# DaehwanKimLab/centrifuge

Hardware: NVIDIA H100
Metric: reads/sec (100 bp SE classification) (higher is better)
Workload: dtype u64

## Files before the change

### centrifuge_b200/capi.py

```python
import ctypes as C
import os

import numpy as np

HERE = os.path.dirname(os.path.abspath(__file__))
LIB_PATH = os.path.join(HERE, "libcfb200.so")

CFB_UID_NONE = 0xFFFFFFFF
REC_DTYPE = np.dtype([("taxid", "<u8"), ("score", "<u4"), ("hitlen", "<u4"), ("uid", "<u4"), ("pad", "<u4")])

_lib = None


class CfbError(RuntimeError):
    pass


class IndexInfo(C.Structure):
    _fields_ = [("len", C.c_uint64), ("num_sides", C.c_uint64), ("n_seqs", C.c_uint64), ("n_tax_nodes", C.c_uint64),
                ("n_boundaries", C.c_uint64), ("line_rate", C.c_int32), ("off_rate", C.c_int32), ("ftab_chars", C.c_int32),
                ("sample_bytes", C.c_int32), ("compressed", C.c_int32), ("device", C.c_int32), ("device_bytes", C.c_uint64)]


class IndexTables(C.Structure):
# ... 280 lines not shown
        out = (C.c_uint64 * 5)()
        _ck(lib().cfb_ctx_requests(self.h, out))
        return dict(zip(["rank16", "ftab2", "ftabk", "walk8", "ftabd"], [int(x) for x in out]))

    def request_breakdown(self):
        out = (C.c_uint64 * 8)()
        _ck(lib().cfb_ctx_request_breakdown(self.h, out))
        names = ["rank16_w1", "rank16_w2_4", "rank16_w5", "walk8_try_row", "walk8_ok_row", "walk8_try_range", "walk8_ok_range", "walk8_ok_w5"]
        return dict(zip(names, [int(x) for x in out]))

    def search_iter_stats(self):
        out = (C.c_uint64 * 8)()
        _ck(lib().cfb_ctx_search_iter_stats(self.h, out))
        names = ["warp_iters", "lane_requests", "consumer_paths", "restart_paths", "task_iters", "clk_head", "clk_wait", "clk_tail"]
        return dict(zip(names, [int(x) for x in out]))

    def counters(self):
        out = (C.c_uint64 * 8)()
        _ck(lib().cfb_ctx_counters(self.h, out))
        names = ["units", "partial_searches", "ftab_probes", "sides_search", "walk_steps", "rows_resolved", "lf_steps", "ext_searches"]
        return dict(zip(names, [int(x) for x in out]))

    def launches(self):
        n = C.c_uint64()
        _ck(lib().cfb_ctx_kernel_launches(self.h, C.byref(n)))
        return int(n.value)

    def close(self):
        if self.h:
            lib().cfb_ctx_destroy(self.h)
# ... 133 lines not shown
```

### centrifuge_b200/csrc/cf_logic.h

```cpp
#ifndef CF_LOGIC_H_
#define CF_LOGIC_H_

#include <stdint.h>

#ifdef __CUDACC__
#define CFB_HD __host__ __device__ __forceinline__
#define CFB_HDN __host__ __device__
#else
#define CFB_HD inline
#define CFB_HDN inline
#endif

namespace cfb {

static const uint64_t kOff = 0xffffffffffffffffull;
static const uint64_t kUnk = 0xfffffffffffffffeull;
static const uint32_t kBwNone = 0xffffffffu;

struct IndexView {
	const uint64_t* sides;
	const uint64_t* ftab;
	const uint64_t* eftab;
	const uint16_t* sample16;
	const uint32_t* sample32;
	const uint64_t* brow;
	const uint32_t* bseq;
	const uint32_t* bbits;
	const uint64_t* seq_taxid;
	const int32_t*  seq_path;
	const uint64_t* paths;
	const uint8_t*  seq_excluded;
	const uint64_t* host_taxids;
	const uint64_t* rank16;
	const uint64_t* ftab2;
	const uint16_t* rtab16;
	const uint32_t* rtab32;
	const uint64_t* ftabk;
	const uint64_t* walk8;
	uint64_t walk8_rows;
	int32_t  ftabd_chars;
	uint64_t len, zoff, zside, fchr[4], last_boundary, num_sides;
	uint32_t zoffc, n_boundaries, n_seqs, n_host;
	int32_t  off_rate, ftab_chars, bshift, ftabk_chars;
};

struct Params {
	uint32_t khits, min_hitlen, ihits, increment;
	uint32_t tree_traverse, class_rank_slot;
};

struct HitRec { uint64_t top, bot; uint32_t bwoff, len; };

static const uint64_t kRowMask = (1ull << 40) - 1ull, kRowStart = 1ull << 63, kRowSameTs = 1ull << 58;

struct Counters {
	unsigned long long units, partial_searches, ftab_probes, sides_search, walk_steps, rows_resolved, lf_steps, ext_searches;
	unsigned long long req_rank16, req_ftab2, req_ftabk, req_walk8, req_ftabd;
	unsigned long long r16_w1, r16_w2_4, r16_w5, w8_try_row, w8_ok_row, w8_try_range, w8_ok_range, w8_ok_w5;
	unsigned long long it_warp, it_lane_req, it_consumers, it_restarts, it_task, clk_head, clk_wait, clk_tail;
};

CFB_HD int popc64(uint64_t x) {
#ifdef __CUDA_ARCH__
	return __popcll(x);
#else
	return __builtin_popcountll(x);
#endif
}
CFB_HD uint32_t ctz32(uint32_t x) {
#ifdef __CUDA_ARCH__
	return (uint32_t)(__ffs(x) - 1);
#else
	return (uint32_t)__builtin_ctz(x);
#endif
// ... 361 lines not shown
			const uint64_t nelt = hsize(L[hi]) < maxG ? hsize(L[hi]) : maxG;
			if(nelt > p.ihits) continue;
			const uint64_t head = kRowStart | ((uint64_t)(L[hi].len & 0xffffu) << 40) | ((uint64_t)(rdi & 1) << 56) | ((uint64_t)(fwi & 1) << 57)
			                    | (ts == last_ts ? kRowSameTs : 0ull);
			last_ts = ts;
			for(uint64_t e = 0; e < nelt; e++) out[k++] = ((L[hi].top + e) & kRowMask) | (e == 0 ? head : 0ull);
			cnt += nelt;
			if(cnt >= maxG) break;
		}
	}
};

static const uint32_t kUidOff = 0xffffffffu;
struct Entry {
	uint64_t taxID;
	uint32_t uniqueID;
	uint32_t scores[2][2], lens[2][2];
	uint32_t score, hitlen, ts;
	int32_t  pid;
	uint8_t  rank;
	uint8_t  pad[3];
};
struct TaxCnt { uint32_t count; uint32_t pad; uint64_t parent; };
struct TaxCntLess { CFB_HD bool operator()(const TaxCnt& a, const TaxCnt& b) const { return a.count < b.count || (a.count == b.count && a.parent < b.parent); } };

struct OutRec { uint64_t taxid; uint32_t score, hitlen, uid, pad; };

CFB_HD bool is_host(const IndexView& v, uint64_t taxid) {
	uint32_t lo = 0, hi = v.n_host;
	while(lo < hi) { uint32_t mid = (lo + hi) >> 1; if(v.host_taxids[mid] < taxid) lo = mid + 1; else hi = mid; }
	return lo < v.n_host && v.host_taxids[lo] == taxid;
}
CFB_HD uint32_t path_size(const Entry& e) { return e.pid < 0 ? 0u : 10u; }
CFB_HD uint64_t path_at(const IndexView& v, const Entry& e, uint32_t i) { return v.paths[(uint64_t)e.pid * 10 + i]; }

CFB_HDN uint32_t score_plan(const IndexView& v, const Params& p, const uint64_t* rows, const uint32_t* ids, uint64_t n, Entry* map) {
	uint32_t nmap = 0, ts = 0;
	for(uint64_t k = 0; k < n;) {
		const uint64_t head = rows[k];
		if(!(head & kRowSameTs)) ts++;
		const uint64_t hl = (head >> 40) & 0xffffu; const int rdi = (int)((head >> 56) & 1), fwi = (int)((head >> 57) & 1);
		uint64_t nelt = 1;
		while(k + nelt < n && !(rows[k + nelt] & kRowStart)) nelt++;
		const uint32_t* my = ids + k; k += nelt;
		const uint32_t sc = (uint32_t)((hl - 15) * (hl - 15));
		for(uint64_t e = 0; e < nelt; e++) {
			const uint32_t ref = my[e];
			bool dup = false;
			for(uint64_t q = 0; q < e; q++) if(my[q] == ref) { dup = true; break; }
			if(dup) continue;
			uint64_t taxID = ref < v.n_seqs ? v.seq_taxid[ref] : 0;
			if(v.seq_excluded && ref < v.n_seqs && v.seq_excluded[ref]) continue;
			const int32_t pid = ref < v.n_seqs ? v.seq_path[ref] : -1;
			uint8_t rank = (uint8_t)p.class_rank_slot;
			if(rank > 0 && pid >= 0) {
				for(; rank < 10; rank++) { const uint64_t t = v.paths[(uint64_t)pid * 10 + rank]; if(t != 0) { taxID = t; break; } }
			}
			uint32_t idx = 0;
			for(; idx < nmap; ++idx) {
				const bool same = rank == 0 ? (ref == map[idx].uniqueID) : (taxID == map[idx].taxID);
				if(same) {
					if(map[idx].ts != ts) { map[idx].scores[rdi][fwi] += sc; map[idx].lens[rdi][fwi] += (uint32_t)hl; map[idx].ts = ts; }
					break;
				}
			}
			if(idx >= nmap) {
				Entry& n2 = map[nmap++];
				n2.uniqueID = ref; n2.taxID = taxID;
				n2.scores[0][0] = n2.scores[0][1] = n2.scores[1][0] = n2.scores[1][1] = 0;
				n2.lens[0][0] = n2.lens[0][1] = n2.lens[1][0] = n2.lens[1][1] = 0;
				n2.scores[rdi][fwi] = sc; n2.lens[rdi][fwi] = (uint32_t)hl;
				n2.score = 0; n2.hitlen = 0; n2.ts = ts; n2.pid = pid; n2.rank = rank;
			}
		}
	}
	return nmap;
}


CFB_HDN uint32_t reduce_and_emit(const IndexView& v, const Params& p, bool paired, Entry* map, uint32_t nmap,
                                 TaxCnt* tc, OutRec* out) {
	const uint32_t k = p.khits;
	for(uint32_t i = 0; i < nmap; i++) {
		Entry& h = map[i];
		const uint32_t s0 = h.scores[0][0] > h.scores[0][1] ? h.scores[0][0] : h.scores[0][1];
		const uint32_t l0 = h.lens[0][0] > h.lens[0][1] ? h.lens[0][0] : h.lens[0][1];
		if(paired) {
			const uint32_t s1 = h.scores[1][0] > h.scores[1][1] ? h.scores[1][0] : h.scores[1][1];
			const uint32_t l1 = h.lens[1][0] > h.lens[1][1] ? h.lens[1][0] : h.lens[1][1];
			h.score = s0 + s1; h.hitlen = l0 + l1;
		} else { h.score = s0; h.hitlen = l0; }
	}
	int64_t best = 0; bool only_host = false;
	for(uint32_t i = 0; i < nmap; i++) {
		if((int64_t)map[i].score > best) { best = map[i].score; only_host = is_host(v, map[i].taxID); }
		else if((int64_t)map[i].score == best) only_host |= is_host(v, map[i].taxID);
	}
	if(!only_host && nmap > k) {
		uint32_t bs = map[0].score;
		for(uint32_t i = 1; i < nmap; i++) if(bs < map[i].score) bs = map[i].score;
		for(int i = 0; i < (int)nmap; i++) {
			if(map[i].score < bs) { if(i + 1 < (int)nmap) map[i] = map[nmap - 1]; nmap--; i--; }
		}
		if(!p.tree_traverse && nmap > k) return 0;
		uint8_t rank = 0;
		while(nmap > k) {
			uint32_t ntc = 0;
			for(uint32_t i = 0; i < nmap; i++) {
				Entry& h = map[i];
				while(h.rank < rank) {
					if((uint32_t)h.rank + 1 >= path_size(h)) { h.rank = 255; break; }
					h.rank += 1; h.taxID = path_at(v, h, h.rank);
				}
				if(h.rank > rank) continue;
				const uint64_t parent = ((uint32_t)rank + 1 >= path_size(h)) ? 1 : path_at(v, h, rank + 1);
				if(parent == 0) continue;
				uint32_t j = 0;
				for(; j < ntc; j++) if(tc[j].parent == parent) { tc[j].count += 1; break; }
				if(j == ntc) { tc[ntc].count = 1; tc[ntc].pad = 0; tc[ntc].parent = parent; ntc++; }
			}
			if(ntc == 0) {
				if(rank < path_size(map[0])) { rank++; continue; } else break;
			}
			ss_heapsort(tc, tc + ntc, TaxCntLess());
			uint32_t j = ntc;
			while(j-- > 0) {
				const uint64_t parent = tc[j].parent;
				for(uint32_t i = 0; i < nmap; i++) {
					Entry& h = map[i];
					if(h.rank != rank) continue;
					const uint64_t cur_parent = ((uint32_t)rank + 1 >= path_size(h)) ? 1 : path_at(v, h, rank + 1);
					if(parent == cur_parent) { h.uniqueID = kUidOff; h.rank = rank + 1; h.taxID = parent; }
				}
				bool first = true;
				for(uint32_t i = 0; i < nmap; i++) {
					if(parent == map[i].taxID) {
						if(!first) { if(i + 1 < nmap) map[i] = map[nmap - 1]; nmap--; i--; }
						else first = false;
					}
				}
				if(nmap <= k) break;
			}
			++rank;
			if(rank > path_size(map[0])) break;
		}
	}
	if(!only_host && nmap > k) return 0;
// ... 34 lines not shown
```

### centrifuge_b200/csrc/cf_multi.cuh

```cuda
#include <dlfcn.h>
#include <nccl.h>

extern "C" int cfb_ctx_count_records(cfb_ctx* c, int on) {
	if(!c) return fail(CFB_EINVAL, "null ctx");
	CK(cudaSetDevice(c->ix->device));
	if(on) { int rc = counts_init(c); if(rc) return rc; }
	c->fold_records = on != 0;
	return CFB_OK;
}
extern "C" int cfb_counts_taxids(cfb_ctx* c, uint64_t* taxid, uint64_t cap, uint64_t* n) {
	if(!c || !n) return fail(CFB_EINVAL, "null argument");
	CK(cudaSetDevice(c->ix->device));
	int rc = counts_init(c); if(rc) return rc;
	*n = c->cnt.n;
	if(taxid) { if(cap < c->cnt.n) return fail(CFB_EINVAL, "cfb_counts_taxids: buffer too small"); memcpy(taxid, c->cnt.h_taxid.data(), (size_t)c->cnt.n * 8); }
	return CFB_OK;
}
extern "C" int cfb_counts_reset(cfb_ctx* c) {
	if(!c) return fail(CFB_EINVAL, "null ctx");
	CK(cudaSetDevice(c->ix->device));
	if(!c->cnt.ready) return CFB_OK;
	CK(cudaDeviceSynchronize());
	CK(cudaMemset(c->cnt.total.p, 0, 3ull * c->cnt.n * 8)); CK(cudaMemset(c->cnt.global.p, 0, 3ull * c->cnt.n * 8));
	c->cnt.reduced = false;
// ... 145 lines not shown
	if(!c || !out) return fail(CFB_EINVAL, "null argument");
	CK(cudaSetDevice(c->ix->device));
	Counters h; CK(cudaMemcpy(&h, c->d_ctr, sizeof h, cudaMemcpyDeviceToHost));
	out[0] = h.r16_w1; out[1] = h.r16_w2_4; out[2] = h.r16_w5;
	out[3] = h.w8_try_row; out[4] = h.w8_ok_row; out[5] = h.w8_try_range; out[6] = h.w8_ok_range; out[7] = h.w8_ok_w5;
	return CFB_OK;
}
extern "C" int cfb_ctx_search_iter_stats(cfb_ctx* c, uint64_t out[8]) {
	if(!c || !out) return fail(CFB_EINVAL, "null argument");
	CK(cudaSetDevice(c->ix->device));
	Counters h; CK(cudaMemcpy(&h, c->d_ctr, sizeof h, cudaMemcpyDeviceToHost));
	out[0] = h.it_warp; out[1] = h.it_lane_req; out[2] = h.it_consumers; out[3] = h.it_restarts; out[4] = h.it_task;
	out[5] = h.clk_head; out[6] = h.clk_wait; out[7] = h.clk_tail;
	return CFB_OK;
}

__device__ __forceinline__ uint64_t gmix(uint64_t x) { x += 0x9E3779B97F4A7C15ull; x = (x ^ (x >> 30)) * 0xBF58476D1CE4E5B9ull; x = (x ^ (x >> 27)) * 0x94D049BB133111EBull; return x ^ (x >> 31); }
template <int W, int ILP>
__global__ void __launch_bounds__(128) k_gather_probe(const unsigned long long* __restrict__ a, uint64_t n, uint32_t iters, unsigned long long* sink) {
	const uint64_t tid = (uint64_t)blockIdx.x * blockDim.x + threadIdx.x;
	uint64_t h = gmix(tid * 0x2545F4914F6CDD1Dull + 1), acc = 0;
	for(uint32_t it = 0; it < iters; it++) {
		unsigned long long v[ILP][W];
		#pragma unroll
		for(int k = 0; k < ILP; k++) {
			h = gmix(h + k);
			const uint64_t u = h % n;
			if(W == 2) { const ulonglong2 q = __ldg(reinterpret_cast<const ulonglong2*>(a) + u); v[k][0] = q.x; v[k][W - 1] = q.y; }
			else v[k][0] = __ldg(a + u);
		}
// ... 42 lines not shown
```

### centrifuge_b200/csrc/cfb200.cu

```cuda
#include "../../include/cfb200.h"
#include "cf_index.h"
#include "cf_kernels.cuh"

#include <algorithm>
#include <atomic>
#include <mutex>
#include <thread>
#include <fcntl.h>
#include <unistd.h>
#include <cstdarg>
#include <cstdio>
#include <cstring>
#include <set>
#include <string>
#include <vector>

using namespace cfb;

enum { M_DONE = 0, M_FTAB = 1, M_LF = 2, M_NEED = 3, M_FTABK = 4, M_TASK = 5 };

struct SearchArgs {
	IndexView v; Params p; BatchView b;
	HitRec* hits; uint32_t* nhits; uint32_t cap;
	unsigned long long* task_ctr64; uint32_t ntasks, chunk;
// ... 594 lines not shown
	}
	const unsigned lane = threadIdx.x & 31;
	uint64_t incl = rows;
	for(int d = 1; d < 32; d <<= 1) { const uint64_t t = __shfl_up_sync(0xffffffffu, incl, d); if((int)lane >= d) incl += t; }
	const uint64_t warp_total = __shfl_sync(0xffffffffu, incl, 31);
	unsigned long long base = 0;
	if(lane == 31 && warp_total) base = atomicAdd(a.row_total, (unsigned long long)warp_total);
	base = __shfl_sync(0xffffffffu, base, 31);
	if(!live) return;
	const uint64_t off = base + incl - rows;
	a.nrows[unit] = (uint32_t)rows; a.row_off[unit] = off;
	if(rows && off + rows <= a.rows_cap) { EmitRows er(a.p, u, a.rows + off); for_each_visit(a.p, u, er); }
}

static const int kScoreThreads = 128;
static const uint32_t kScorePool = 128;
static const uint32_t kNoSlot = 0xffffffffu;
template <int MINB>
__global__ void __launch_bounds__(kScoreThreads, MINB) k_score(const UnitArgs a) {
	__shared__ uint64_t s_rows[kScorePool]; __shared__ uint32_t s_ids[kScorePool];
	__shared__ Entry s_map[kScorePool]; __shared__ TaxCnt s_tc[kScorePool]; __shared__ OutRec s_recs[kScorePool];
	__shared__ uint32_t s_used;
	if(threadIdx.x == 0) s_used = 0;
	__syncthreads();
	const uint32_t unit = blockIdx.x * blockDim.x + threadIdx.x;
	const unsigned lane = threadIdx.x & 31;
	const bool valid = unit < a.b.n_units;
	const bool fits = *a.row_total <= a.rows_cap;
	const uint64_t n = valid && fits ? a.nrows[unit] : 0, off = valid && fits ? a.row_off[unit] : 0;
	const uint64_t base = __shfl_sync(0xffffffffu, off, 0);
	uint64_t span = n ? off + n - base : 0;
	for(int d = 16; d > 0; d >>= 1) span = max(span, __shfl_xor_sync(0xffffffffu, span, d));
	uint32_t slot = kNoSlot;
	if(lane == 0 && span) {
		uint32_t cur = *(volatile uint32_t*)&s_used;
		while(span <= kScorePool - cur) {
			const uint32_t old = atomicCAS(&s_used, cur, cur + (uint32_t)span);
			if(old == cur) { slot = cur; break; }
			cur = old;
		}
	}
	slot = __shfl_sync(0xffffffffu, slot, 0);
	const bool sh = slot != kNoSlot;
	if(sh) {
		for(uint32_t j = lane; j < (uint32_t)span; j += 32) { s_rows[slot + j] = a.rows[base + j]; s_ids[slot + j] = a.ids[base + j]; }
		__syncwarp();
	}
	const uint32_t loc = sh ? slot + (uint32_t)(off - base) : 0u;
	uint32_t no = 0;
	if(n > 0) {
		const uint8_t fl = a.b.flags ? a.b.flags[unit] : 3;
		int mates = 0;
		for(int m = 0; m < a.b.n_mates; m++) if(((fl >> m) & 1) && (m ? a.b.len[1][unit] : a.b.len[0][unit]) != 0) mates++;
		const uint64_t* rows = sh ? s_rows + loc : a.rows + off;
		const uint32_t* ids = sh ? s_ids + loc : a.ids + off;
		Entry* map = sh ? s_map + loc : a.entries + off;
		TaxCnt* tc = sh ? s_tc + loc : a.tcs + off;
		OutRec* out = sh ? s_recs + loc : a.recs_sparse + off;
		const uint32_t nmap = score_plan(a.v, a.p, rows, ids, n, map);
		no = reduce_and_emit(a.v, a.p, mates == 2, map, nmap, tc, out);
	}
	if(valid) a.nout[unit] = no;
	if(sh) {
		__syncwarp();
		for(int u = 0; u < 32; u++) {
			const uint32_t cnt = __shfl_sync(0xffffffffu, no, u) * 3u, l = __shfl_sync(0xffffffffu, loc, u);
			const uint64_t o = __shfl_sync(0xffffffffu, off, u);
			const uint64_t* src = reinterpret_cast<const uint64_t*>(s_recs + l);
			uint64_t* dst = reinterpret_cast<uint64_t*>(a.recs_sparse + o);
			for(uint32_t w = lane; w < cnt; w += 32) dst[w] = src[w];
		}
	}
}

static const int kScanBlock = 256, kScanPer = 4;

__global__ void __launch_bounds__(kScanBlock) k_scan_sums(const uint32_t* in, uint64_t n, uint64_t* bsum) {
	__shared__ uint64_t sh[kScanBlock];
	const uint64_t base = (uint64_t)blockIdx.x * kScanBlock * kScanPer + (uint64_t)threadIdx.x * kScanPer;
	uint64_t s = 0;
	for(int i = 0; i < kScanPer; i++) if(base + i < n) s += in[base + i];
	sh[threadIdx.x] = s; __syncthreads();
	for(int d = kScanBlock / 2; d > 0; d >>= 1) { if((int)threadIdx.x < d) sh[threadIdx.x] += sh[threadIdx.x + d]; __syncthreads(); }
	if(threadIdx.x == 0) bsum[blockIdx.x] = sh[0];
}
__global__ void k_scan_top(uint64_t* bsum, uint64_t nb, uint64_t* total) {
	__shared__ uint64_t carry;
// ... 380 lines not shown
	if(!p) return;
	memset(p, 0, sizeof *p); p->khits = 5; p->min_hitlen = 22; p->tree_traverse = 1; p->class_rank_slot = 0;
}

static const int kSlots = 17;

struct Slot {
	cudaStream_t st = nullptr;
	cudaEvent_t ev[6] = {nullptr, nullptr, nullptr, nullptr, nullptr, nullptr};
	HBuf<uint8_t> h_bases; HBuf<uint64_t> h_off; HBuf<uint32_t> h_len; HBuf<uint8_t> h_flags;
	DBuf<uint8_t> d_bases; DBuf<uint64_t> d_off; DBuf<uint32_t> d_len; DBuf<uint8_t> d_flags;
	HBuf<uint64_t> h_words; DBuf<uint64_t> d_words, d_npos, d_woff; DBuf<uint32_t> d_wlen;
	DBuf<uint64_t> pk; DBuf<uint32_t> nm;
	DBuf<HitRec> hits; DBuf<uint32_t> nhits; DBuf<HitRec> regen; DBuf<uint32_t> regen_n; uint64_t regen_slots = 0; uint32_t full_cap = 0; DBuf<uint32_t> nrows; DBuf<uint64_t> row_off; DBuf<uint64_t> bsum;
	DBuf<uint64_t> rows; DBuf<uint32_t> ids; DBuf<Entry> entries; DBuf<TaxCnt> tcs; DBuf<OutRec> sparse;
	DBuf<uint32_t> nout; DBuf<uint64_t> out_off; DBuf<OutRec> dense; DBuf<uint32_t> rec_off32;
	DBuf<unsigned long long> scal;
	HBuf<unsigned long long> h_scal;
	HBuf<OutRec> h_recs; HBuf<uint32_t> h_rec_off;
	DBuf<unsigned long long> cnt;
	bool folded = false, is_text = false, commit_pending = false;
	BatchView bv; uint64_t n_units = 0, n_bases = 0; uint32_t maxlen = 0, cap = 0; uint64_t rows_cap = 0, dense_cap = 0;
	bool pending = false, reran = false;
	bool want_host = false; uint64_t d2h_recs = 0;
	void release() {
		h_bases.release(); h_off.release(); h_len.release(); h_flags.release(); d_bases.release(); d_off.release(); d_len.release(); d_flags.release();
		h_words.release(); d_words.release(); d_npos.release(); d_woff.release(); d_wlen.release();
		pk.release(); nm.release(); hits.release(); nhits.release(); regen.release(); regen_n.release(); nrows.release(); row_off.release(); bsum.release(); rows.release(); ids.release(); entries.release(); tcs.release();
		sparse.release(); nout.release(); out_off.release(); dense.release(); rec_off32.release(); scal.release(); h_scal.release(); h_recs.release(); h_rec_off.release(); cnt.release();
		for(int i = 0; i < 6; i++) if(ev[i]) cudaEventDestroy(ev[i]);
		if(st) cudaStreamDestroy(st);
	}
};

struct cfb_dbatch { int slot; uint64_t n_units; };
struct TextCtx;
static void text_release(cfb_ctx*);
static void comm_release(cfb_ctx*);

struct CountsCtx {
	bool ready = false;
	std::vector<uint64_t> h_taxid; DBuf<uint64_t> d_taxid; uint32_t n = 0;
	DBuf<unsigned long long> total, global; bool reduced = false;
	void release() { d_taxid.release(); total.release(); global.release(); }
};

struct cfb_ctx {
	const cfb_index* ix = nullptr;
	IndexView view; Params prm;
	DBuf<uint8_t> d_excl; DBuf<uint64_t> d_host;
	Slot slots[kSlots];
	Counters* d_ctr = nullptr; int count = 0;
	uint64_t launches = 0;
	int resolve_blocks = 0;
	cfb_dbatch resident; bool resident_used = false;
	double rec_ratio = 2.0;
	uint64_t rows_cap0 = 0;
	TextCtx* text = nullptr;
	CountsCtx cnt; bool fold_records = false;
	bool keep_short = false;
	uint64_t regen_lists = 0, regen_tasks = 0;
	uint64_t regen_slots0 = 0;
	void* comm = nullptr; int comm_rank = 0, comm_size = 1; cudaStream_t comm_st = nullptr;
};

// ... 10 lines not shown
			t = nd->parent;
		}
	}
}

extern "C" void cfb_ctx_destroy(cfb_ctx* c) {
	if(!c) return;
	if(c->ix && c->ix->device >= 0) cudaSetDevice(c->ix->device);
	if(getenv("CFB_REGEN_STATS") && c->regen_tasks)
		fprintf(stderr, "[cfb] strand lists regenerated by k_prep: %llu of %llu (%.3f %%)\n", (unsigned long long)c->regen_lists,
		        (unsigned long long)c->regen_tasks, 100.0 * (double)c->regen_lists / (double)c->regen_tasks);
	text_release(c);
	comm_release(c);
	c->cnt.release();
	for(int i = 0; i < kSlots; i++) c->slots[i].release();
	c->d_excl.release(); c->d_host.release();
	if(c->d_ctr) cudaFree(c->d_ctr);
	delete c;
}

extern "C" int cfb_ctx_create(const cfb_index* ix, const cfb_params* p, cfb_ctx** out) {
	if(!ix || !p || !out) return fail(CFB_EINVAL, "cfb_ctx_create: null argument");
	if(ix->device < 0) return fail(CFB_ENODEV, "index was loaded host-only; classification needs a CUDA device (no CPU fallback)");
	if(p->khits < 1) return fail(CFB_EINVAL, "khits must be >= 1");
	CK(cudaSetDevice(ix->device));
	cfb_ctx* c = new cfb_ctx();
	c->ix = ix; c->view = ix->view;
	const HostIndex& h = ix->h;
	Params& q = c->prm;
	q.khits = (uint32_t)p->khits;
	q.min_hitlen = (uint32_t)(p->min_hitlen < 15 ? 15 : p->min_hitlen);
	q.ihits = (uint32_t)std::max(p->khits, 5) * (h.compressed ? 4u : 40u);
	q.increment = (2 * q.min_hitlen <= 33) ? 10 : (2 * q.min_hitlen - 33);
	q.tree_traverse = p->tree_traverse ? 1 : 0;
	q.class_rank_slot = (uint32_t)(p->class_rank_slot & 0xff);
	std::set<uint64_t> host, excl;
	expand_taxids(h, p->host_taxids, p->n_host_taxids, host);
	expand_taxids(h, p->excluded_taxids, p->n_excluded_taxids, excl);
	#define CKC(call) do { cudaError_t e_ = (call); if(e_ != cudaSuccess) { cfb_ctx_destroy(c); return fail(CFB_ECUDA, "%s failed: %s", #call, cudaGetErrorString(e_)); } } while(0)
	if(!excl.empty()) {
		std::vector<uint8_t> fl(h.seq_taxid.size(), 0);
		for(size_t i = 0; i < fl.size(); i++) fl[i] = excl.count(h.seq_taxid[i]) ? 1 : 0;
		CKC(c->d_excl.ensure(fl.size())); CKC(cudaMemcpy(c->d_excl.p, fl.data(), fl.size(), cudaMemcpyHostToDevice));
		c->view.seq_excluded = c->d_excl.p;
	}
	if(!host.empty()) {
		std::vector<uint64_t> hv(host.begin(), host.end());
		CKC(c->d_host.ensure(hv.size())); CKC(cudaMemcpy(c->d_host.p, hv.data(), hv.size() * 8, cudaMemcpyHostToDevice));
		c->view.host_taxids = c->d_host.p; c->view.n_host = (uint32_t)hv.size();
	}
	for(int i = 0; i < kSlots; i++) {
		CKC(cudaStreamCreateWithFlags(&c->slots[i].st, cudaStreamNonBlocking));
		for(int e = 0; e < 6; e++) CKC(cudaEventCreate(&c->slots[i].ev[e]));
		CKC(c->slots[i].scal.ensure(8)); CKC(c->slots[i].h_scal.ensure(8));
	}
	CKC(cudaMalloc((void**)&c->d_ctr, sizeof(Counters))); CKC(cudaMemset(c->d_ctr, 0, sizeof(Counters)));
	cudaDeviceSetLimit(cudaLimitMaxL2FetchGranularity, 32);
	cudaGetLastError();
	int occ = 0;
// ... 212 lines not shown
	const SearchKernel search = search_kernel(s.maxlen, c->count);
	const bool keep_short = search == k_search_long<true> || search == k_search_long<false> || c->prm.min_hitlen < kLongLen || c->keep_short;
	if(stage == 0) {
		if(s.cap == 0) {
			s.full_cap = s.maxlen / 4 + 8;
			s.cap = keep_short ? s.full_cap : s.maxlen / kLongLen + 2;
		}
		CK(s.hits.ensure(ntasks * s.cap)); CK(s.nhits.ensure(ntasks));
		if(!keep_short) {
			s.regen_slots = std::max<uint64_t>(s.regen_slots, c->regen_slots0 ? c->regen_slots0 : std::max<uint64_t>(ntasks / 32, 1024));
			CK(s.regen.ensure(s.regen_slots * s.full_cap)); CK(s.regen_n.ensure(s.regen_slots));
			CK(cudaMemsetAsync(s.scal.p + 6, 0, sizeof(unsigned long long), s.st));
		}
		const uint32_t W = (s.maxlen + 31) / 32 + 1;
		CK(s.pk.ensure(ntasks * W + 2)); CK(s.nm.ensure(ntasks * W + 2)); CK(s.nrows.ensure(n)); CK(s.row_off.ensure(n + 1));
		CK(s.bsum.ensure(scan_blocks + 1)); CK(s.nout.ensure(n)); CK(s.out_off.ensure(n + 1)); CK(s.rec_off32.ensure(n + 1));
		s.rows_cap = std::max<uint64_t>(s.rows_cap, c->rows_cap0 ? c->rows_cap0 : std::max<uint64_t>(n * 12, 4096));
	}
	CK(s.rows.ensure(s.rows_cap)); CK(s.ids.ensure(s.rows_cap)); CK(s.entries.ensure(s.rows_cap)); CK(s.tcs.ensure(s.rows_cap)); CK(s.sparse.ensure(s.rows_cap));
	s.dense_cap = s.rows_cap; CK(s.dense.ensure(s.dense_cap));
	CK(cudaMemsetAsync(s.scal.p, 0, 4 * sizeof(unsigned long long), s.st));
	if(time_it) CK(cudaEventRecord(s.ev[0], s.st));
	Counters* ctr = c->count ? c->d_ctr : nullptr;
	if(c->count && stage == 0) CK(cudaMemsetAsync(c->d_ctr, 0, sizeof(Counters), s.st));
	UnitArgs ua; ua.v = c->view; ua.p = c->prm; ua.b = s.bv; ua.hits = s.hits.p; ua.nhits = s.nhits.p; ua.cap = s.cap;
	ua.nrows = s.nrows.p; ua.row_off = s.row_off.p; ua.row_total = s.scal.p + 3; ua.rows = s.rows.p; ua.ids = s.ids.p; ua.rows_cap = s.rows_cap;
	ua.entries = s.entries.p; ua.tcs = s.tcs.p; ua.recs_sparse = s.sparse.p; ua.nout = s.nout.p;
	ua.overflow = (unsigned int*)(s.scal.p + 2); ua.ctr = ctr;
	ua.regen = s.regen.p; ua.regen_n = s.regen_n.p; ua.regen_ctr = s.scal.p + 6; ua.regen_slots = s.regen_slots; ua.full_cap = s.full_cap; ua.keep_short = keep_short ? 1u : 0u;
	if(stage == 0) {
		SearchArgs sa; sa.v = c->view; sa.p = c->prm; sa.b = s.bv; sa.hits = s.hits.p; sa.nhits = s.nhits.p; sa.cap = s.cap;
		const uint32_t W = (s.maxlen + 31) / 32 + 1;
		sa.pk = s.pk.p; sa.nm = s.nm.p; sa.W = W; sa.keep_short = keep_short ? 1u : 0u;
		{ PackArgs pa; pa.b = s.bv; pa.pk = s.pk.p; pa.nm = s.nm.p; pa.W = W;
		  k_pack<<<(unsigned)((ntasks * W + 127) / 128), 128, 0, s.st>>>(pa); c->launches++; }
		sa.task_ctr64 = s.scal.p + 0; sa.ntasks = (uint32_t)ntasks; sa.overflow = (unsigned int*)(s.scal.p + 2); sa.ctr = ctr;
		int occ = 1;
		CK(cudaOccupancyMaxActiveBlocksPerMultiprocessor(&occ, search, kSearchThreads, 0));
		const uint64_t resident = (uint64_t)c->ix->sm_count * (uint64_t)std::max(occ, 1);
// ... 4 lines not shown
		c->launches++;
		if(time_it) CK(cudaEventRecord(s.ev[1], s.st));
		k_prep<8, false><<<ublocks, 128, 0, s.st>>>(ua); c->launches++;
	} else {
		if(time_it) CK(cudaEventRecord(s.ev[1], s.st));
		k_prep<8, true><<<ublocks, 128, 0, s.st>>>(ua); c->launches++;
	}
	if(time_it) CK(cudaEventRecord(s.ev[2], s.st));
	ResolveArgs ra; ra.v = c->view; ra.rows = s.rows.p; ra.ids = s.ids.p; ra.ids16 = nullptr; ra.total = (const uint64_t*)(s.scal.p + 3); ra.rows_cap = s.rows_cap;
	ra.task_ctr = s.scal.p + 1; ra.chunk = 64; ra.ctr = ctr;
	if((c->view.rtab16 || c->view.rtab32) && c->count != 1) k_lookup<<<c->ix->sm_count * 8, 256, 0, s.st>>>(ra);
	else if(c->count) k_resolve_c<true, false><<<c->resolve_blocks, kSearchThreads, 0, s.st>>>(ra);
	else k_resolve_c<false, false><<<c->resolve_blocks, kSearchThreads, 0, s.st>>>(ra);
	c->launches++;
	if(time_it) CK(cudaEventRecord(s.ev[3], s.st));
	k_score<12><<<ublocks, kScoreThreads, 0, s.st>>>(ua); c->launches++;
	k_scan_sums<<<(unsigned)scan_blocks, kScanBlock, 0, s.st>>>(s.nout.p, n, s.bsum.p);
	k_scan_top<<<1, 1024, 0, s.st>>>(s.bsum.p, scan_blocks, (uint64_t*)(s.scal.p + 4));
	k_scan_apply<<<(unsigned)scan_blocks, kScanBlock, 0, s.st>>>(s.nout.p, n, s.bsum.p, (const uint64_t*)(s.scal.p + 4), s.out_off.p);
	k_compact<<<(unsigned)((n + 1 + 127) / 128), 128, 0, s.st>>>((uint32_t)n, s.row_off.p, s.out_off.p, s.sparse.p, s.dense.p, s.rec_off32.p, s.dense_cap, (unsigned int*)(s.scal.p + 2));
	c->launches += 4;
	s.folded = false;
	if(c->fold_records && !s.is_text) {
		const uint32_t nsp = c->cnt.n;
		CK(s.cnt.ensure(3ull * nsp)); CK(cudaMemsetAsync(s.cnt.p, 0, 3ull * nsp * 8, s.st));
		FoldArgs fa; fa.sp_taxid = c->cnt.d_taxid.p; fa.n_sp = nsp; fa.rec_off = s.rec_off32.p; fa.recs = s.dense.p; fa.n_units = (uint32_t)n; fa.n_mates = nm;
		fa.khits = c->prm.khits; fa.len[0] = s.bv.len[0]; fa.len[1] = s.bv.len[1]; fa.flags = s.bv.flags; fa.sp = s.cnt.p;
		k_fold_counts<<<ublocks, 128, 0, s.st>>>(fa); c->launches++;
		s.folded = true;
	}
	if(time_it) CK(cudaEventRecord(s.ev[4], s.st));
	s.d2h_recs = 0;
	if(s.want_host) {
		const uint64_t guess = std::min<uint64_t>(s.dense_cap, (uint64_t)((double)n * c->rec_ratio * 1.05) + 4096);
// ... 198 lines not shown
```

### include/cfb200.h

```cpp
#ifndef CFB200_H_
#define CFB200_H_

#include <stddef.h>
#include <stdint.h>

#ifdef __cplusplus
extern "C" {
#endif

#define CFB_OK        0
#define CFB_EINVAL   -1
#define CFB_EIO      -2
#define CFB_ENOMEM   -3
#define CFB_ENODEV   -4
#define CFB_ECUDA    -5
#define CFB_EFORMAT  -6

#define CFB_UID_NONE 0xFFFFFFFFu

typedef struct cfb_index cfb_index;
typedef struct cfb_ctx   cfb_ctx;

int cfb_index_load(const char* basename, int device, cfb_index** out);
#define CFB_LOAD_NO_RESOLVE_TABLE 1u
// ... 117 lines not shown
int cfb_counts_reset(cfb_ctx*);
int cfb_counts_read(cfb_ctx*, int global, uint64_t* taxid, uint64_t* n_reads, uint64_t* n_unique, uint64_t* n_obs1, uint64_t cap, uint64_t* n);
int cfb_counts_dense(cfb_ctx*, int global, uint64_t* out, uint64_t cap);
#define CFB_COMM_ID_BYTES 128
int cfb_comm_unique_id(uint8_t id[CFB_COMM_ID_BYTES]);
int cfb_comm_init_rank(cfb_ctx*, int nranks, int rank, const uint8_t id[CFB_COMM_ID_BYTES]);
int cfb_comm_init_all(cfb_ctx* const* ctxs, int n);
int cfb_comm_info(const cfb_ctx*, int* rank, int* size, int* nccl_version);
int cfb_counts_allreduce(cfb_ctx* const* ctxs, int n, uint64_t* dense_out, uint64_t cap);

int cfb_ctx_requests(cfb_ctx*, uint64_t out[5]);
int cfb_ctx_request_breakdown(cfb_ctx*, uint64_t out[8]);
int cfb_gather_ceiling(const cfb_index*, int table, uint64_t n_requests, double* g_requests_per_s, double* ms);
int cfb_gather_rate(const cfb_index*, int table, uint64_t n_requests, int ctas_per_sm, int ilp, double* g_requests_per_s, double* ms);
int cfb_ctx_search_iter_stats(cfb_ctx*, uint64_t out[8]);

int cfb_ctx_counters(cfb_ctx*, uint64_t out[8]);
int cfb_ctx_kernel_launches(const cfb_ctx*, uint64_t* n);

int   cfb_device_count(void);
void* cfb_host_alloc(size_t bytes);
void  cfb_host_free(void*);

int cfb_test_lf(const cfb_index*, const uint64_t* rows, const uint8_t* chars, uint64_t n, uint64_t* out);
int cfb_test_resolve(const cfb_index*, const uint64_t* rows, uint64_t n, uint32_t* out);
int cfb_test_parse(const char* path, int fasta, int trim5, int trim3, uint32_t seed, const char* out_path);
int cfb_test_host_path(const char* index_base, const char* reads_a, const char* reads_b, int fasta, int khits, uint32_t seed,
                       int trim5, int trim3, const uint32_t* rec_off, const cfb_rec* recs, uint64_t n_units,
                       const char* out_tsv, const char* out_report, const char* out_kreport);

// ... 41 lines not shown
```

Before: 293.1 million.

## Precompute per-sequence info table, slim score kernel shared memory, use CUB scan

Builds a per-sequence SeqInfo table on the host (taxid, path id, excluded flag, resolved rank) so score_plan does one 16-byte load instead of several scattered loads plus a path walk. The score kernel now keeps only the Entry map in shared memory, with a larger pool, and reads rows, ids and output records directly from global memory, dropping the staging copies. Parent taxids are cached in the entries so the tree-reduce loop stops re-reading paths. The three-kernel custom scan is replaced by a CUB exclusive scan, and optional score-stage counters are added behind a template flag.

```diff
diff --git a/centrifuge_b200/capi.py b/centrifuge_b200/capi.py
--- a/centrifuge_b200/capi.py
+++ b/centrifuge_b200/capi.py
@@ -318,6 +318,15 @@
         _ck(lib().cfb_ctx_search_iter_stats(self.h, out))
         names = ["warp_iters", "lane_requests", "consumer_paths", "restart_paths", "task_iters", "clk_head", "clk_wait", "clk_tail"]
         return dict(zip(names, [int(x) for x in out]))
+
+    def score_stats(self):
+        out = (C.c_uint64 * 23)()
+        _ck(lib().cfb_ctx_score_stats(self.h, out))
+        v = [int(x) for x in out]
+        names = ["units", "rows", "distinct_ids", "reduce_units", "reduce_rounds", "warps", "warps_global"]
+        d = dict(zip(names, v[:7]))
+        d["rows_hist"], d["distinct_ids_hist"] = v[7:15], v[15:23]
+        return d
 
     def counters(self):
         out = (C.c_uint64 * 8)()
diff --git a/centrifuge_b200/csrc/cf_logic.h b/centrifuge_b200/csrc/cf_logic.h
--- a/centrifuge_b200/csrc/cf_logic.h
+++ b/centrifuge_b200/csrc/cf_logic.h
@@ -16,6 +16,13 @@
 static const uint64_t kOff = 0xffffffffffffffffull;
 static const uint64_t kUnk = 0xfffffffffffffffeull;
 static const uint32_t kBwNone = 0xffffffffu;
+
+struct alignas(16) SeqInfo {
+	uint64_t taxid;
+	int32_t  pid;
+	uint32_t flags;
+};
+static const uint32_t kSeqExcluded = 1u;
 
 struct IndexView {
 	const uint64_t* sides;
@@ -31,6 +38,7 @@
 	const uint64_t* paths;
 	const uint8_t*  seq_excluded;
 	const uint64_t* host_taxids;
+	const SeqInfo*  seqs;
 	const uint64_t* rank16;
 	const uint64_t* ftab2;
 	const uint16_t* rtab16;
@@ -58,6 +66,8 @@
 	unsigned long long req_rank16, req_ftab2, req_ftabk, req_walk8, req_ftabd;
 	unsigned long long r16_w1, r16_w2_4, r16_w5, w8_try_row, w8_ok_row, w8_try_range, w8_ok_range, w8_ok_w5;
 	unsigned long long it_warp, it_lane_req, it_consumers, it_restarts, it_task, clk_head, clk_wait, clk_tail;
+	unsigned long long sc_units, sc_rows, sc_nmap, sc_reduce, sc_rounds, sc_warps, sc_warps_global;
+	unsigned long long sc_rows_hist[8], sc_nmap_hist[8];
 };
 
 CFB_HD int popc64(uint64_t x) {
@@ -449,8 +459,12 @@
 static const uint32_t kUidOff = 0xffffffffu;
 struct Entry {
 	uint64_t taxID;
+	union {
+		uint32_t scores[2][2];
+		uint64_t parent;
+	};
+	uint32_t lens[2][2];
 	uint32_t uniqueID;
-	uint32_t scores[2][2], lens[2][2];
 	uint32_t score, hitlen, ts;
 	int32_t  pid;
 	uint8_t  rank;
@@ -467,7 +481,31 @@
 	return lo < v.n_host && v.host_taxids[lo] == taxid;
 }
 CFB_HD uint32_t path_size(const Entry& e) { return e.pid < 0 ? 0u : 10u; }
-CFB_HD uint64_t path_at(const IndexView& v, const Entry& e, uint32_t i) { return v.paths[(uint64_t)e.pid * 10 + i]; }
+CFB_HD uint64_t path_at(const IndexView& v, const Entry& e, uint32_t i) {
+#ifdef __CUDA_ARCH__
+	return __ldg(v.paths + (uint64_t)e.pid * 10 + i);
+#else
+	return v.paths[(uint64_t)e.pid * 10 + i];
+#endif
+}
+
+CFB_HD SeqInfo seq_info_of(const IndexView& v, const Params& p, uint32_t ref) {
+	SeqInfo s; s.taxid = 0; s.pid = -1;
+	uint32_t rank = p.class_rank_slot & 0xffu, excl = 0;
+	if(ref < v.n_seqs) {
+		s.taxid = v.seq_taxid[ref]; s.pid = v.seq_path[ref];
+		excl = v.seq_excluded && v.seq_excluded[ref] ? kSeqExcluded : 0u;
+		if(rank > 0 && s.pid >= 0) {
+			for(; rank < 10; rank++) { const uint64_t t = v.paths[(uint64_t)s.pid * 10 + rank]; if(t != 0) { s.taxid = t; break; } }
+		}
+	}
+	s.flags = excl | rank << 8;
+	return s;
+}
+CFB_HD SeqInfo seq_info(const IndexView& v, const Params& p, uint32_t ref) {
+	if(v.seqs && ref < v.n_seqs) return v.seqs[ref];
+	return seq_info_of(v, p, ref);
+}
 
 CFB_HDN uint32_t score_plan(const IndexView& v, const Params& p, const uint64_t* rows, const uint32_t* ids, uint64_t n, Entry* map) {
 	uint32_t nmap = 0, ts = 0;
@@ -484,13 +522,9 @@
 			bool dup = false;
 			for(uint64_t q = 0; q < e; q++) if(my[q] == ref) { dup = true; break; }
 			if(dup) continue;
-			uint64_t taxID = ref < v.n_seqs ? v.seq_taxid[ref] : 0;
-			if(v.seq_excluded && ref < v.n_seqs && v.seq_excluded[ref]) continue;
-			const int32_t pid = ref < v.n_seqs ? v.seq_path[ref] : -1;
-			uint8_t rank = (uint8_t)p.class_rank_slot;
-			if(rank > 0 && pid >= 0) {
-				for(; rank < 10; rank++) { const uint64_t t = v.paths[(uint64_t)pid * 10 + rank]; if(t != 0) { taxID = t; break; } }
-			}
+			const SeqInfo si = seq_info(v, p, ref);
+			if(si.flags & kSeqExcluded) continue;
+			const uint64_t taxID = si.taxid; const int32_t pid = si.pid; const uint8_t rank = (uint8_t)(si.flags >> 8);
 			uint32_t idx = 0;
 			for(; idx < nmap; ++idx) {
 				const bool same = rank == 0 ? (ref == map[idx].uniqueID) : (taxID == map[idx].taxID);
@@ -512,9 +546,9 @@
 	return nmap;
 }
 
-
 CFB_HDN uint32_t reduce_and_emit(const IndexView& v, const Params& p, bool paired, Entry* map, uint32_t nmap,
-                                 TaxCnt* tc, OutRec* out) {
+                                 TaxCnt* tc, OutRec* out, uint32_t* rounds = nullptr) {
+	if(rounds) *rounds = 0;
 	const uint32_t k = p.khits;
 	for(uint32_t i = 0; i < nmap; i++) {
 		Entry& h = map[i];
@@ -540,15 +574,20 @@
 		if(!p.tree_traverse && nmap > k) return 0;
 		uint8_t rank = 0;
 		while(nmap > k) {
-			uint32_t ntc = 0;
+			if(rounds) *rounds += 1;
 			for(uint32_t i = 0; i < nmap; i++) {
 				Entry& h = map[i];
 				while(h.rank < rank) {
 					if((uint32_t)h.rank + 1 >= path_size(h)) { h.rank = 255; break; }
 					h.rank += 1; h.taxID = path_at(v, h, h.rank);
 				}
-				if(h.rank > rank) continue;
-				const uint64_t parent = ((uint32_t)rank + 1 >= path_size(h)) ? 1 : path_at(v, h, rank + 1);
+				if(h.rank == rank) h.parent = ((uint32_t)rank + 1 >= path_size(h)) ? 1 : path_at(v, h, rank + 1);
+			}
+			uint32_t ntc = 0;
+			for(uint32_t i = 0; i < nmap; i++) {
+				const Entry& h = map[i];
+				if(h.rank != rank) continue;
+				const uint64_t parent = h.parent;
 				if(parent == 0) continue;
 				uint32_t j = 0;
 				for(; j < ntc; j++) if(tc[j].parent == parent) { tc[j].count += 1; break; }
@@ -563,9 +602,7 @@
 				const uint64_t parent = tc[j].parent;
 				for(uint32_t i = 0; i < nmap; i++) {
 					Entry& h = map[i];
-					if(h.rank != rank) continue;
-					const uint64_t cur_parent = ((uint32_t)rank + 1 >= path_size(h)) ? 1 : path_at(v, h, rank + 1);
-					if(parent == cur_parent) { h.uniqueID = kUidOff; h.rank = rank + 1; h.taxID = parent; }
+					if(h.rank == rank && h.parent == parent) { h.uniqueID = kUidOff; h.rank = rank + 1; h.taxID = parent; }
 				}
 				bool first = true;
 				for(uint32_t i = 0; i < nmap; i++) {
diff --git a/centrifuge_b200/csrc/cf_multi.cuh b/centrifuge_b200/csrc/cf_multi.cuh
--- a/centrifuge_b200/csrc/cf_multi.cuh
+++ b/centrifuge_b200/csrc/cf_multi.cuh
@@ -183,6 +183,14 @@
 	out[5] = h.clk_head; out[6] = h.clk_wait; out[7] = h.clk_tail;
 	return CFB_OK;
 }
+extern "C" int cfb_ctx_score_stats(cfb_ctx* c, uint64_t out[23]) {
+	if(!c || !out) return fail(CFB_EINVAL, "null argument");
+	CK(cudaSetDevice(c->ix->device));
+	Counters h; CK(cudaMemcpy(&h, c->d_ctr, sizeof h, cudaMemcpyDeviceToHost));
+	out[0] = h.sc_units; out[1] = h.sc_rows; out[2] = h.sc_nmap; out[3] = h.sc_reduce; out[4] = h.sc_rounds; out[5] = h.sc_warps; out[6] = h.sc_warps_global;
+	for(int i = 0; i < 8; i++) { out[7 + i] = h.sc_rows_hist[i]; out[15 + i] = h.sc_nmap_hist[i]; }
+	return CFB_OK;
+}
 
 __device__ __forceinline__ uint64_t gmix(uint64_t x) { x += 0x9E3779B97F4A7C15ull; x = (x ^ (x >> 30)) * 0xBF58476D1CE4E5B9ull; x = (x ^ (x >> 27)) * 0x94D049BB133111EBull; return x ^ (x >> 31); }
 template <int W, int ILP>
diff --git a/centrifuge_b200/csrc/cfb200.cu b/centrifuge_b200/csrc/cfb200.cu
--- a/centrifuge_b200/csrc/cfb200.cu
+++ b/centrifuge_b200/csrc/cfb200.cu
@@ -1,6 +1,7 @@
 #include "../../include/cfb200.h"
 #include "cf_index.h"
 #include "cf_kernels.cuh"
+#include <cub/cub.cuh>
 
 #include <algorithm>
 #include <atomic>
@@ -632,12 +633,12 @@
 }
 
 static const int kScoreThreads = 128;
-static const uint32_t kScorePool = 128;
+static const uint32_t kScorePool = 232;
 static const uint32_t kNoSlot = 0xffffffffu;
-template <int MINB>
+__device__ __forceinline__ uint32_t log2_bucket(uint64_t x) { const uint32_t b = 63u - (uint32_t)__clzll((long long)x); return b < 7u ? b : 7u; }
+template <int MINB, bool COUNT>
 __global__ void __launch_bounds__(kScoreThreads, MINB) k_score(const UnitArgs a) {
-	__shared__ uint64_t s_rows[kScorePool]; __shared__ uint32_t s_ids[kScorePool];
-	__shared__ Entry s_map[kScorePool]; __shared__ TaxCnt s_tc[kScorePool]; __shared__ OutRec s_recs[kScorePool];
+	__shared__ Entry s_map[kScorePool];
 	__shared__ uint32_t s_used;
 	if(threadIdx.x == 0) s_used = 0;
 	__syncthreads();
@@ -660,35 +661,24 @@
 	}
 	slot = __shfl_sync(0xffffffffu, slot, 0);
 	const bool sh = slot != kNoSlot;
-	if(sh) {
-		for(uint32_t j = lane; j < (uint32_t)span; j += 32) { s_rows[slot + j] = a.rows[base + j]; s_ids[slot + j] = a.ids[base + j]; }
-		__syncwarp();
-	}
-	const uint32_t loc = sh ? slot + (uint32_t)(off - base) : 0u;
 	uint32_t no = 0;
 	if(n > 0) {
 		const uint8_t fl = a.b.flags ? a.b.flags[unit] : 3;
 		int mates = 0;
 		for(int m = 0; m < a.b.n_mates; m++) if(((fl >> m) & 1) && (m ? a.b.len[1][unit] : a.b.len[0][unit]) != 0) mates++;
-		const uint64_t* rows = sh ? s_rows + loc : a.rows + off;
-		const uint32_t* ids = sh ? s_ids + loc : a.ids + off;
-		Entry* map = sh ? s_map + loc : a.entries + off;
-		TaxCnt* tc = sh ? s_tc + loc : a.tcs + off;
-		OutRec* out = sh ? s_recs + loc : a.recs_sparse + off;
-		const uint32_t nmap = score_plan(a.v, a.p, rows, ids, n, map);
-		no = reduce_and_emit(a.v, a.p, mates == 2, map, nmap, tc, out);
-	}
+		Entry* map = sh ? s_map + slot + (uint32_t)(off - base) : a.entries + off;
+		const uint32_t nmap = score_plan(a.v, a.p, a.rows + off, a.ids + off, n, map);
+		uint32_t rounds = 0;
+		no = reduce_and_emit(a.v, a.p, mates == 2, map, nmap, a.tcs + off, a.recs_sparse + off, COUNT ? &rounds : nullptr);
+		if(COUNT) {
+			atomicAdd(&a.ctr->sc_units, 1ull); atomicAdd(&a.ctr->sc_rows, (unsigned long long)n); atomicAdd(&a.ctr->sc_nmap, (unsigned long long)nmap);
+			atomicAdd(&a.ctr->sc_rows_hist[log2_bucket(n)], 1ull);
+			if(nmap) atomicAdd(&a.ctr->sc_nmap_hist[log2_bucket(nmap)], 1ull);
+			if(rounds) { atomicAdd(&a.ctr->sc_reduce, 1ull); atomicAdd(&a.ctr->sc_rounds, (unsigned long long)rounds); }
+		}
+	}
+	if(COUNT && lane == 0 && span) { atomicAdd(&a.ctr->sc_warps, 1ull); if(!sh) atomicAdd(&a.ctr->sc_warps_global, 1ull); }
 	if(valid) a.nout[unit] = no;
-	if(sh) {
-		__syncwarp();
-		for(int u = 0; u < 32; u++) {
-			const uint32_t cnt = __shfl_sync(0xffffffffu, no, u) * 3u, l = __shfl_sync(0xffffffffu, loc, u);
-			const uint64_t o = __shfl_sync(0xffffffffu, off, u);
-			const uint64_t* src = reinterpret_cast<const uint64_t*>(s_recs + l);
-			uint64_t* dst = reinterpret_cast<uint64_t*>(a.recs_sparse + o);
-			for(uint32_t w = lane; w < cnt; w += 32) dst[w] = src[w];
-		}
-	}
 }
 
 static const int kScanBlock = 256, kScanPer = 4;
@@ -1099,7 +1089,7 @@
 	DBuf<uint64_t> pk; DBuf<uint32_t> nm;
 	DBuf<HitRec> hits; DBuf<uint32_t> nhits; DBuf<HitRec> regen; DBuf<uint32_t> regen_n; uint64_t regen_slots = 0; uint32_t full_cap = 0; DBuf<uint32_t> nrows; DBuf<uint64_t> row_off; DBuf<uint64_t> bsum;
 	DBuf<uint64_t> rows; DBuf<uint32_t> ids; DBuf<Entry> entries; DBuf<TaxCnt> tcs; DBuf<OutRec> sparse;
-	DBuf<uint32_t> nout; DBuf<uint64_t> out_off; DBuf<OutRec> dense; DBuf<uint32_t> rec_off32;
+	DBuf<uint32_t> nout; DBuf<uint64_t> out_off; DBuf<uint8_t> scan_tmp; DBuf<OutRec> dense; DBuf<uint32_t> rec_off32;
 	DBuf<unsigned long long> scal;
 	HBuf<unsigned long long> h_scal;
 	HBuf<OutRec> h_recs; HBuf<uint32_t> h_rec_off;
@@ -1112,7 +1102,7 @@
 		h_bases.release(); h_off.release(); h_len.release(); h_flags.release(); d_bases.release(); d_off.release(); d_len.release(); d_flags.release();
 		h_words.release(); d_words.release(); d_npos.release(); d_woff.release(); d_wlen.release();
 		pk.release(); nm.release(); hits.release(); nhits.release(); regen.release(); regen_n.release(); nrows.release(); row_off.release(); bsum.release(); rows.release(); ids.release(); entries.release(); tcs.release();
-		sparse.release(); nout.release(); out_off.release(); dense.release(); rec_off32.release(); scal.release(); h_scal.release(); h_recs.release(); h_rec_off.release(); cnt.release();
+		sparse.release(); nout.release(); out_off.release(); scan_tmp.release(); dense.release(); rec_off32.release(); scal.release(); h_scal.release(); h_recs.release(); h_rec_off.release(); cnt.release();
 		for(int i = 0; i < 6; i++) if(ev[i]) cudaEventDestroy(ev[i]);
 		if(st) cudaStreamDestroy(st);
 	}
@@ -1133,7 +1123,7 @@
 struct cfb_ctx {
 	const cfb_index* ix = nullptr;
 	IndexView view; Params prm;
-	DBuf<uint8_t> d_excl; DBuf<uint64_t> d_host;
+	DBuf<uint64_t> d_host; DBuf<SeqInfo> d_seqs;
 	Slot slots[kSlots];
 	Counters* d_ctr = nullptr; int count = 0;
 	uint64_t launches = 0;
@@ -1174,7 +1164,7 @@
 	comm_release(c);
 	c->cnt.release();
 	for(int i = 0; i < kSlots; i++) c->slots[i].release();
-	c->d_excl.release(); c->d_host.release();
+	c->d_host.release(); c->d_seqs.release();
 	if(c->d_ctr) cudaFree(c->d_ctr);
 	delete c;
 }
@@ -1198,11 +1188,19 @@
 	expand_taxids(h, p->host_taxids, p->n_host_taxids, host);
 	expand_taxids(h, p->excluded_taxids, p->n_excluded_taxids, excl);
 	#define CKC(call) do { cudaError_t e_ = (call); if(e_ != cudaSuccess) { cfb_ctx_destroy(c); return fail(CFB_ECUDA, "%s failed: %s", #call, cudaGetErrorString(e_)); } } while(0)
+	std::vector<uint8_t> fl;
 	if(!excl.empty()) {
-		std::vector<uint8_t> fl(h.seq_taxid.size(), 0);
+		fl.assign(h.seq_taxid.size(), 0);
 		for(size_t i = 0; i < fl.size(); i++) fl[i] = excl.count(h.seq_taxid[i]) ? 1 : 0;
-		CKC(c->d_excl.ensure(fl.size())); CKC(cudaMemcpy(c->d_excl.p, fl.data(), fl.size(), cudaMemcpyHostToDevice));
-		c->view.seq_excluded = c->d_excl.p;
+	}
+	{
+		IndexView hv; memset(&hv, 0, sizeof hv);
+		hv.seq_taxid = h.seq_taxid.data(); hv.seq_path = h.seq_path.data(); hv.paths = h.paths.data(); hv.n_seqs = (uint32_t)h.seq_taxid.size();
+		hv.seq_excluded = fl.empty() ? nullptr : fl.data();
+		std::vector<SeqInfo> tab(hv.n_seqs);
+		for(uint32_t i = 0; i < hv.n_seqs; i++) tab[i] = seq_info_of(hv, q, i);
+		CKC(c->d_seqs.ensure(tab.size() + 1)); CKC(cudaMemcpy(c->d_seqs.p, tab.data(), tab.size() * sizeof(SeqInfo), cudaMemcpyHostToDevice));
+		c->view.seqs = c->d_seqs.p;
 	}
 	if(!host.empty()) {
 		std::vector<uint64_t> hv(host.begin(), host.end());
@@ -1445,7 +1443,7 @@
 		}
 		const uint32_t W = (s.maxlen + 31) / 32 + 1;
 		CK(s.pk.ensure(ntasks * W + 2)); CK(s.nm.ensure(ntasks * W + 2)); CK(s.nrows.ensure(n)); CK(s.row_off.ensure(n + 1));
-		CK(s.bsum.ensure(scan_blocks + 1)); CK(s.nout.ensure(n)); CK(s.out_off.ensure(n + 1)); CK(s.rec_off32.ensure(n + 1));
+		CK(s.bsum.ensure(scan_blocks + 1)); CK(s.nout.ensure(n + 1)); CK(s.out_off.ensure(n + 1)); CK(s.rec_off32.ensure(n + 1));
 		s.rows_cap = std::max<uint64_t>(s.rows_cap, c->rows_cap0 ? c->rows_cap0 : std::max<uint64_t>(n * 12, 4096));
 	}
 	CK(s.rows.ensure(s.rows_cap)); CK(s.ids.ensure(s.rows_cap)); CK(s.entries.ensure(s.rows_cap)); CK(s.tcs.ensure(s.rows_cap)); CK(s.sparse.ensure(s.rows_cap));
@@ -1454,6 +1452,10 @@
 	if(time_it) CK(cudaEventRecord(s.ev[0], s.st));
 	Counters* ctr = c->count ? c->d_ctr : nullptr;
 	if(c->count && stage == 0) CK(cudaMemsetAsync(c->d_ctr, 0, sizeof(Counters), s.st));
+	else if(c->count) {
+		const size_t sc0 = offsetof(Counters, sc_units);
+		CK(cudaMemsetAsync(reinterpret_cast<char*>(c->d_ctr) + sc0, 0, sizeof(Counters) - sc0, s.st));
+	}
 	UnitArgs ua; ua.v = c->view; ua.p = c->prm; ua.b = s.bv; ua.hits = s.hits.p; ua.nhits = s.nhits.p; ua.cap = s.cap;
 	ua.nrows = s.nrows.p; ua.row_off = s.row_off.p; ua.row_total = s.scal.p + 3; ua.rows = s.rows.p; ua.ids = s.ids.p; ua.rows_cap = s.rows_cap;
 	ua.entries = s.entries.p; ua.tcs = s.tcs.p; ua.recs_sparse = s.sparse.p; ua.nout = s.nout.p;
@@ -1488,10 +1490,14 @@
 	else k_resolve_c<false, false><<<c->resolve_blocks, kSearchThreads, 0, s.st>>>(ra);
 	c->launches++;
 	if(time_it) CK(cudaEventRecord(s.ev[3], s.st));
-	k_score<12><<<ublocks, kScoreThreads, 0, s.st>>>(ua); c->launches++;
-	k_scan_sums<<<(unsigned)scan_blocks, kScanBlock, 0, s.st>>>(s.nout.p, n, s.bsum.p);
-	k_scan_top<<<1, 1024, 0, s.st>>>(s.bsum.p, scan_blocks, (uint64_t*)(s.scal.p + 4));
-	k_scan_apply<<<(unsigned)scan_blocks, kScanBlock, 0, s.st>>>(s.nout.p, n, s.bsum.p, (const uint64_t*)(s.scal.p + 4), s.out_off.p);
+	if(ctr) k_score<12, true><<<ublocks, kScoreThreads, 0, s.st>>>(ua);
+	else k_score<12, false><<<ublocks, kScoreThreads, 0, s.st>>>(ua);
+	size_t scan_bytes = 0;
+	CK(cub::DeviceScan::ExclusiveScan(nullptr, scan_bytes, s.nout.p, s.out_off.p, cub::Sum(), (uint64_t)0, (int)(n + 1), s.st));
+	CK(s.scan_tmp.ensure(scan_bytes));
+	CK(cudaMemsetAsync(s.nout.p + n, 0, sizeof(uint32_t), s.st));
+	CK(cub::DeviceScan::ExclusiveScan(s.scan_tmp.p, scan_bytes, s.nout.p, s.out_off.p, cub::Sum(), (uint64_t)0, (int)(n + 1), s.st));
+	CK(cudaMemcpyAsync(s.scal.p + 4, s.out_off.p + n, sizeof(uint64_t), cudaMemcpyDeviceToDevice, s.st));
 	k_compact<<<(unsigned)((n + 1 + 127) / 128), 128, 0, s.st>>>((uint32_t)n, s.row_off.p, s.out_off.p, s.sparse.p, s.dense.p, s.rec_off32.p, s.dense_cap, (unsigned int*)(s.scal.p + 2));
 	c->launches += 4;
 	s.folded = false;
diff --git a/include/cfb200.h b/include/cfb200.h
--- a/include/cfb200.h
+++ b/include/cfb200.h
@@ -155,6 +155,7 @@
 int cfb_gather_ceiling(const cfb_index*, int table, uint64_t n_requests, double* g_requests_per_s, double* ms);
 int cfb_gather_rate(const cfb_index*, int table, uint64_t n_requests, int ctas_per_sm, int ilp, double* g_requests_per_s, double* ms);
 int cfb_ctx_search_iter_stats(cfb_ctx*, uint64_t out[8]);
+int cfb_ctx_score_stats(cfb_ctx*, uint64_t out[23]);
 
 int cfb_ctx_counters(cfb_ctx*, uint64_t out[8]);
 int cfb_ctx_kernel_launches(const cfb_ctx*, uint64_t* n);
```

Result: faster. 307.7 million, median of 6 (+5.0%).
